# shiyao-li/NextBestPath

Hardware: AMD Instinct MI355X
Metric: exploration steps/s (+ NBP maps/s) at 256x256 (higher is better)
Workload: dtype f32

## Files before the change

### nextbestpath_amd/csrc/nbp_internal.h

```cpp
#pragma once
#include "common.h"

typedef unsigned short bf16_t;

enum { NBP_TILE_AUTO = 0, NBP_TILE_128x128 = 1, NBP_TILE_256x64 = 2, NBP_TILE_256x32 = 3, NBP_TILE_128x64 = 4,
       NBP_TILE_64x128 = 5,
       NBP_TILE_HALO_128 = 6, NBP_TILE_HALO_64 = 7,
       NBP_TILE_HALO4_128 = 8, NBP_TILE_HALO4_64 = 9,
       NBP_TILE_SPLIT_HALO_64 = 10, NBP_TILE_SPLIT_UP = 11,
       NBP_TILE_HALO_UP_128 = 12, NBP_TILE_HALO_UP_64 = 13,
       NBP_TILE_RESERVED_14 = 14,
       NBP_TILE_SPLIT_HALO_R8 = 15, NBP_TILE_SPLIT_UP_R8 = 16,
       NBP_TILE_SPLIT_UP_DGRAD = 17,
       NBP_TILE_SPLIT_HALO_128 = 18,
       NBP_TILE_SPLIT_GATE = 19 };
struct TileInfo { int bm, bn; };
struct ConvPlan { int tile; int split_k; int chunks_per_split; };

struct IgemmArgs {
    const float* src0;
    const float* src1;
    int C0, C1;
    int cc0;
    int ups;
    int H, W;
    int Hs, Ws;
    int taps;
    const float* wpk;
    int N;
    const float* scale;
    const float* shift;
    int relu;
    float* out;
    long long M;
    int split_k;
    int chunks_total;
    int chunks_per_split;
    unsigned bytes0, bytes1;
    unsigned bytesw;
    float* partial;
    int groups;
    const float* g_src0;
    const float* g_src1;
    const float* g_wpk;
    const float* g_scale;
    const float* g_shift;
    float* g_out;
    int xcd_remap;
};
struct ConvOperands { const float* src0; const float* src1; const float* wpk; const float* scale; const float* shift; float* out; };
// ... 59 lines not shown
```

### nextbestpath_amd/csrc/nbp_split.hip

```cpp
#include "common.h"
#include "nbp_internal.h"
#include <cstdlib>

namespace {

typedef _Float16 f16x8 __attribute__((ext_vector_type(8)));
typedef _Float16 f16x2 __attribute__((ext_vector_type(2)));
typedef unsigned u32x4 __attribute__((ext_vector_type(4)));
typedef unsigned u32x2 __attribute__((ext_vector_type(2)));
typedef __attribute__((address_space(3))) void* lds_ptr_t;

constexpr int SPLIT_EXP = 14;
__host__ __device__ inline int amax_exponent(unsigned bits) {
    if (!bits) return SPLIT_EXP;
    int e = (int)((bits >> 23) & 255u) - 127;
    return e < -100 ? -100 : (e > 100 ? 100 : e);
}
__host__ __device__ inline float pow2f(int e) {
    union { unsigned u; float f; } v;
    v.u = (unsigned)(127 + e) << 23;
    return v.f;
}

__device__ __forceinline__ void split_pair(float x0, float x1, unsigned& h, unsigned& l) {
// ... 17 lines not shown
}
__device__ __forceinline__ void block_amax(float mx, unsigned* out, unsigned words = AMAX_WORDS) {
    __shared__ float part[4];
#pragma unroll
    for (int o = 32; o; o >>= 1) mx = fmaxf(mx, __shfl_xor(mx, o));
    if ((threadIdx.x & 63) == 0) part[threadIdx.x >> 6] = mx;
    __syncthreads();
    if (threadIdx.x == 0)
        atomicMax(out + (blockIdx.x & (words - 1)), __float_as_uint(fmaxf(fmaxf(part[0], part[1]), fmaxf(part[2], part[3]))));
}
__device__ __forceinline__ unsigned read_amax(const unsigned* slot) {
    unsigned v = slot[threadIdx.x & (AMAX_WORDS - 1)];
#pragma unroll
    for (int o = 32; o; o >>= 1) { const unsigned u = __shfl_xor(v, o); v = u > v ? u : v; }
    return v;
}

struct SplitOps {
    const float* src0; const float* src1; const void* planes; const float* scale; const float* shift; float* out;
    const unsigned* amax0; const unsigned* amax1; const unsigned* wamax; unsigned* amax_out;
    float* pool_out;
    const float* head_w; const float* head_ss[2]; float* head_out;
    double* bn_part;
    const float* psi0;
};
struct SplitArgs {
    SplitOps g[2];
    int C0, C1, ups, H, W, Hs, Ws, N, relu;
    long long M;
    int split_k, chunks_total, chunks_per_split;
    unsigned bytes0, bytes1, bytesw;
    float* partial;
    int groups, xcd_remap;
};

#ifdef NBP_DBG_TS
__device__ unsigned long long nbp_dbg_ts[8192];
__device__ unsigned nbp_dbg_n;
#define NBP_WALL(tag) do { if (dbg_on) { const unsigned k_ = dbg_i++; if (k_ < 4000) { nbp_dbg_ts[2 * k_] = (unsigned long long)(tag); nbp_dbg_ts[2 * k_ + 1] = wall_clock64(); } } } while (0)
#define NBP_TS(tag) do { if (dbg_on) { const unsigned k_ = dbg_i++; if (k_ < 4000) { nbp_dbg_ts[2 * k_] = (unsigned long long)(tag); nbp_dbg_ts[2 * k_ + 1] = __builtin_readcyclecounter(); } } } while (0)
#else
#define NBP_TS(tag) do {} while (0)
#endif
template <bool ONE, int TW, int TM, int TN, bool PH, bool BS = false, bool P2 = false, bool DG = false>
__global__ __launch_bounds__(256, 2) __attribute__((amdgpu_waves_per_eu(2, 2))) void conv3x3_halo_h2_kernel(SplitArgs a) {
    static_assert(!P2 || PH, "two-parity form: up_conv layers");
    static_assert(!DG || (PH && !BS && !P2), "data gradient of an up_conv layer: the one-parity tap structure");
    constexpr bool PHO = PH && !DG;
    int zs = blockIdx.z;
    const int py = PHO ? (P2 ? zs & 1 : (zs >> 1) & 1) : 0, px = (PHO && !P2) ? zs & 1 : 0;
    if (PHO) zs >>= (P2 ? 1 : 2);
    const int zslice = zs;
    const SplitOps& o = zs >= a.split_k ? a.g[1] : a.g[0];
    if (zs >= a.split_k) zs -= a.split_k;
    constexpr int ROWS = PH ? 2 : 3, TPR = PH ? 2 : 3, TAPS = ROWS * TPR;
    constexpr int BN = TN * 32, NB = BN / 64;
    constexpr int RPB = 32 / TW, TH = 4 * TM * RPB;
    constexpr int HW_ = TW + 2, HPIX = (TH + 2) * HW_;
    constexpr int RS = (HPIX + 7) / 8 * 8 * 16 + 64;
    constexpr int NPL = ONE ? 1 : 2;
    constexpr int HALO_BYTES = 2 * NPL * RS;
    constexpr int WI = TPR * 2 * NPL * NB;
    constexpr int NPAR = P2 ? 2 : 1;
    constexpr int WB1 = WI * 1024, WB = NPAR * WB1;
    constexpr int NF = (HPIX * 4 + 255) / 256;
    static_assert(BN % 64 == 0 && (TH == 16 || TH == 8), "tile shape");
    extern __shared__ __attribute__((aligned(16))) char ldsb[];
    char* const halo = ldsb;
    char* const wbuf = ldsb + HALO_BYTES;
    float* const psil = reinterpret_cast<float*>(ldsb + HALO_BYTES + 2 * WB);

    const int tid = threadIdx.x, lane = tid & 63, wave = tid >> 6;
#ifdef NBP_DBG_TS
    const bool dbg_on = blockIdx.x == gridDim.x / 2 && blockIdx.y == 0 && blockIdx.z == 0 && tid == 64;
    unsigned dbg_i = 0;
    NBP_WALL(100); NBP_TS(101);
#endif
    const int Ht = PHO ? a.Hs : a.H, Wt = PHO ? a.Ws : a.W;
    const int tiles_x = Wt / TW, tiles_y = Ht / TH;
    unsigned tile = blockIdx.x, nt = blockIdx.y;
    if (a.xcd_remap == 1) {
        const unsigned L = blockIdx.x + gridDim.x * blockIdx.y, T = gridDim.x * gridDim.y;
        const unsigned xcd = L & 7u, idx = L >> 3, q = T >> 3, r = T & 7u;
        const unsigned v = xcd * q + min(xcd, r) + idx;
        nt = v % gridDim.y;
        tile = v / gridDim.y;
    } else if (a.xcd_remap == 2) {
// ... 226 lines not shown
#pragma unroll
                for (int j = 0; j < TN; ++j)
#pragma unroll
                    for (int p = 0; p < 2; ++p)
                        wp[j][p] = *reinterpret_cast<const u32x4*>(Bt + ((tt * 4 + p * 2) * NB + (j >> 1)) * 1024 + (j & 1) * 512);
                constexpr int PX[3] = {1, 0, 0};
                constexpr int PW[3] = {0, 1, 0};
#pragma unroll
                for (int v = 0; v < 3; ++v)
#pragma unroll
                    for (int j = 0; j < TN; ++j)
#pragma unroll
                        for (int i = 0; i < TM; ++i)
                            acc[i][j] = __builtin_amdgcn_mfma_f32_32x32x16_f16(__builtin_bit_cast(f16x8, xp[i][PX[v]]),
                                                                               __builtin_bit_cast(f16x8, wp[j][PW[v]]), acc[i][j], 0, 0, 0);
            }
            }
            NBP_TS(2);
            asm volatile("s_waitcnt vmcnt(0)" ::: "memory");
            NBP_TS(3);
            __syncthreads();
            NBP_TS(4);
        }
        if (more) {
            __builtin_amdgcn_s_setprio(0);
            store_halo(c + 1);
            NBP_TS(5);
            __syncthreads();
            NBP_TS(6);
            __builtin_amdgcn_s_setprio(2);
        }
    }

    const bool final_out = (a.split_k == 1);
    float* outp = final_out ? o.out : a.partial + (long long)zslice * a.M * a.N;
    float mx = 0.f;
    constexpr int PS = PHO ? 2 : 1;
    const long long e0 = (PHO ? ((long long)b * a.H + 2 * y0 + py) * a.W + 2 * x0 : ((long long)b * a.H + y0) * a.W + x0) * a.N + n0;
    const long long erem = (a.M * a.N - e0) * 4;
    const __amdgpu_buffer_rsrc_t rso = __builtin_amdgcn_make_buffer_rsrc(outp + e0, 0, erem < 0x7fffffffll ? (int)erem : 0x7fffffff, 0x00020000);
    const unsigned vout = (unsigned)(((TM * wave * RPB * PS * a.W + 4 * khalf * PS) * a.N + (lane & 31)) * 4);
    constexpr bool HEADABLE = !PH && TN == 2;
    const bool head = HEADABLE && final_out && o.head_out;
    const bool bn_stats = BS && final_out && o.bn_part;
    double* const bsh = reinterpret_cast<double*>(ldsb);
    if constexpr (BS) { if (bn_stats) __syncthreads(); }
    double bs1[BS ? TN : 1], bs2[BS ? TN : 1];
#pragma unroll
    for (int j = 0; j < (BS ? TN : 1); ++j) { bs1[j] = 0.0; bs2[j] = 0.0; }
    float hp[HEADABLE ? TM : 1][16];
    if constexpr (HEADABLE) {
#pragma unroll
        for (int i = 0; i < TM; ++i)
#pragma unroll
            for (int r = 0; r < 16; ++r) hp[i][r] = 0.f;
    }
#pragma unroll
    for (int pq = 0; pq < NPAR; ++pq)
#pragma unroll
    for (int j = 0; j < TN; ++j) {
        const int pxe = P2 ? pq : px;
        const int n = n0 + j * 32 + (lane & 31);
        float sc = 1.f, sh = 0.f;
        if (final_out) { sc = o.scale[n]; sh = o.shift[n]; }
        const float hw = head ? o.head_w[n] : 0.f;
        float vals[TM][16];
#pragma unroll
        for (int i = 0; i < TM; ++i) {
#pragma unroll
            for (int r = 0; r < 16; ++r) {
                const int q = (r & 3) + 8 * (r >> 2);
                const unsigned soff = (unsigned)((((i * RPB + q / TW) * PS * a.W + (q % TW) * PS + (PHO ? pxe : 0)) * a.N + j * 32) * 4);
                float v = ldexpf(accs[pq][i][j][r], einv) * sc + sh;
                if (final_out && a.relu) v = fmaxf(v, 0.f);
                mx = fmaxf(mx, fabsf(v));
                if (!head) __builtin_amdgcn_raw_buffer_store_b32(__builtin_bit_cast(unsigned, v), rso, vout, soff, 0);
                vals[i][r] = v;
                if constexpr (HEADABLE) hp[i][r] = fmaf(v, hw, hp[i][r]);
            }
        }
        if constexpr (BS) {
            if (bn_stats) {
#pragma unroll
                for (int i = 0; i < TM; ++i)
#pragma unroll
                    for (int r = 0; r < 16; ++r) { const double d = (double)vals[i][r]; bs1[j] += d; bs2[j] = fma(d, d, bs2[j]); }
            }
        }
        if (!PH && final_out && o.pool_out) {
            const int Hp = a.H >> 1, Wp = a.W >> 1;
            if constexpr (TW == 32) {
#pragma unroll
                for (int i = 0; i < TM; i += 2) {
                    const long long prow = ((long long)b * Hp + ((y0 + TM * wave + i) >> 1)) * Wp + (x0 >> 1);
#pragma unroll
                    for (int r = 0; r < 16; r += 2) {
                        const int xo = ((r & 3) + 8 * (r >> 2) + 4 * khalf) >> 1;
                        o.pool_out[(prow + xo) * a.N + n] = fmaxf(fmaxf(vals[i][r], vals[i][r + 1]), fmaxf(vals[i + 1][r], vals[i + 1][r + 1]));
                    }
                }
            } else {
#pragma unroll
                for (int i = 0; i < TM; ++i) {
                    const long long prow = ((long long)b * Hp + ((y0 + (TM * wave + i) * RPB) >> 1)) * Wp + (x0 >> 1);
#pragma unroll
                    for (int r = 0; r < 8; r += 2) {
// ... 681 lines not shown
    const unsigned stride = gridDim.x * 256u * 4u;
    float mx = 0.f;
    for (unsigned i0 = (blockIdx.x * 256u + threadIdx.x) * 4u; i0 < MN; i0 += 2 * stride) {
        const unsigned i1 = i0 + stride;
        const bool two = i1 < MN;
        f32x4 v0 = *reinterpret_cast<const f32x4*>(partial + i0);
        f32x4 v1 = two ? *reinterpret_cast<const f32x4*>(partial + i1) : f32x4{0.f, 0.f, 0.f, 0.f};
        for (int s0 = 1; s0 < split_k; s0 += 4) {
            f32x4 u0[4], u1[4];
#pragma unroll
            for (int k = 0; k < 4; ++k) {
                const bool in = s0 + k < split_k;
                const float* ps = partial + (size_t)(s0 + k) * MN;
                u0[k] = in ? *reinterpret_cast<const f32x4*>(ps + i0) : f32x4{0.f, 0.f, 0.f, 0.f};
                u1[k] = in && two ? *reinterpret_cast<const f32x4*>(ps + i1) : f32x4{0.f, 0.f, 0.f, 0.f};
            }
#pragma unroll
            for (int k = 0; k < 4; ++k)
                if (s0 + k < split_k) {
#pragma unroll
                    for (int e = 0; e < 4; ++e) { v0[e] += u0[k][e]; v1[e] += u1[k][e]; }
                }
        }
#pragma unroll
        for (int h = 0; h < 2; ++h) {
            if (h && !two) break;
            const unsigned i = h ? i1 : i0;
            f32x4 v = h ? v1 : v0;
            const unsigned n = i % N;
            const f32x4 sc = *reinterpret_cast<const f32x4*>(scale + n);
            const f32x4 sh = *reinterpret_cast<const f32x4*>(shift + n);
#pragma unroll
            for (int e = 0; e < 4; ++e) {
                v[e] = v[e] * sc[e] + sh[e];
                if (relu) v[e] = fmaxf(v[e], 0.f);
                mx = fmaxf(mx, fabsf(v[e]));
            }
            *reinterpret_cast<f32x4*>(out + i) = v;
        }
    }
    if (amax_out) block_amax(mx, amax_out);
}

__global__ __launch_bounds__(256) void splitk_reduce_pool_kernel(const float* __restrict__ partial, int split_k, unsigned MN, unsigned N,
                                                                 int H, int W, SplitOps o, int relu) {
    const unsigned N4 = N >> 2, Wp = (unsigned)W >> 1, Hp = (unsigned)H >> 1;
    const unsigned total = (MN >> 4);
    const unsigned rowN = (unsigned)W * N;
    float mx = 0.f;
    for (unsigned p = blockIdx.x * 256u + threadIdx.x; p < total; p += gridDim.x * 256u) {
        const unsigned n4 = p % N4;
        unsigned q = p / N4;
        const unsigned xp = q % Wp; q /= Wp;
        const unsigned yp = q % Hp, b = q / Hp;
        const unsigned base = ((b * (unsigned)H + 2u * yp) * (unsigned)W + 2u * xp) * N + 4u * n4;
        const unsigned idx[4] = {base, base + N, base + rowN, base + rowN + N};
        f32x4 v[4];
#pragma unroll
        for (int k = 0; k < 4; ++k) v[k] = *reinterpret_cast<const f32x4*>(partial + idx[k]);
        for (int s0 = 1; s0 < split_k; s0 += 2) {
            f32x4 u[2][4];
#pragma unroll
            for (int t = 0; t < 2; ++t) {
                const bool in = s0 + t < split_k;
                const float* ps = partial + (size_t)(s0 + t) * MN;
#pragma unroll
                for (int k = 0; k < 4; ++k) u[t][k] = in ? *reinterpret_cast<const f32x4*>(ps + idx[k]) : f32x4{0.f, 0.f, 0.f, 0.f};
            }
#pragma unroll
            for (int t = 0; t < 2; ++t)
                if (s0 + t < split_k) {
#pragma unroll
                    for (int k = 0; k < 4; ++k)
#pragma unroll
                        for (int e = 0; e < 4; ++e) v[k][e] += u[t][k][e];
                }
        }
        const f32x4 sc = *reinterpret_cast<const f32x4*>(o.scale + 4u * n4);
        const f32x4 sh = *reinterpret_cast<const f32x4*>(o.shift + 4u * n4);
        f32x4 pm;
#pragma unroll
        for (int k = 0; k < 4; ++k) {
#pragma unroll
            for (int e = 0; e < 4; ++e) {
                float r = v[k][e] * sc[e] + sh[e];
                if (relu) r = fmaxf(r, 0.f);
                mx = fmaxf(mx, fabsf(r));
                v[k][e] = r;
                pm[e] = k ? fmaxf(pm[e], r) : r;
            }
            *reinterpret_cast<f32x4*>(o.out + idx[k]) = v[k];
        }
        *reinterpret_cast<f32x4*>(o.pool_out + 4u * p) = pm;
    }
    if (o.amax_out) block_amax(mx, o.amax_out);
}

__global__ __launch_bounds__(256) void amax_kernel(const float* __restrict__ x, long long n, const float* __restrict__ row_scale,
                                                   long long per_row, unsigned* __restrict__ out, unsigned words) {
    float mx = 0.f;
    if (!row_scale && (n & 3) == 0 && ((uintptr_t)x & 15) == 0) {
        for (long long i = (long long)blockIdx.x * blockDim.x + threadIdx.x; i < n / 4; i += (long long)gridDim.x * blockDim.x) {
            const f32x4 v = reinterpret_cast<const f32x4*>(x)[i];
            mx = fmaxf(fmaxf(mx, fmaxf(fabsf(v[0]), fabsf(v[1]))), fmaxf(fabsf(v[2]), fabsf(v[3])));
        }
    } else {
        for (long long i = (long long)blockIdx.x * blockDim.x + threadIdx.x; i < n; i += (long long)gridDim.x * blockDim.x)
            mx = fmaxf(mx, fabsf(row_scale ? x[i] * row_scale[i / per_row] : x[i]));
    }
    block_amax(mx, out, words);
}

template <bool ONE = false>
__global__ void pack_conv_weight_h2_kernel(const float* __restrict__ w, int N, int C, int taps, const float* __restrict__ scale,
                                           int c_off, const unsigned* __restrict__ wamax, unsigned short* __restrict__ dst,
                                           int transposed = 0) {
    const float sw = pow2f(SPLIT_EXP - amax_exponent(*wamax));
    const long long total = (long long)N * C * taps;
// ... 204 lines not shown
            constexpr int NPL = ONE ? 1 : 2;
            e.planes = d.planes + (long long)ph * (C >> 4) * 4 * 2 * NPL * N * 8;
            if (d.planes_t) e.planes_t = d.planes_t + (long long)ph * (N >> 4) * 4 * 2 * NPL * C * 8;
            prepack_store_block<ONE>(e, hl, n8, c8, tap, d.planes_t ? (1 - r) * 2 + (1 - tt) : -1, 4);
        }
        return;
    }
    const int taps = d.kind == 0 ? 9 : 1;
    const long long total = (long long)N8 * C8 * taps;
    for (long long i = (long long)blockIdx.x * blockDim.x + threadIdx.x; i < total; i += (long long)gridDim.x * blockDim.x) {
        const int tap = (int)(i % taps);
        const long long t = i / taps;
        const int c8 = (int)(t % C8), n8 = (int)(t / C8);
        unsigned hl[8][8];
#pragma unroll
        for (int nn = 0; nn < 8; ++nn)
#pragma unroll
            for (int cc = 0; cc < 8; ++cc) {
                unsigned h, l;
                split_pair(d.w[((long long)(n8 * 8 + nn) * C + c8 * 8 + cc) * taps + tap] * swf, 0.f, h, l);
                hl[nn][cc] = (h & 0xffffu) | (l << 16);
            }
        prepack_store_block<ONE>(d, hl, n8, c8, tap, d.planes_t ? taps - 1 - tap : -1, taps);
    }
}

int split_tile_width(int H, int W, int N, int ksize) {
    if (ksize != 3 || H < 16 || H % 16) return 0;
    if (W >= 32 && W % 32 == 0 && N % 64 == 0) return 32;
    if (W >= 16 && W % 16 == 0 && N % 128 == 0) return 16;
    return 0;
}

template <int TW, int TM, int TN, bool PH, bool BS = false, bool P2 = false, bool DG = false, bool ONE = false>
int launch_h2(const SplitArgs& a, hipStream_t st, int tile) {
    {
        char nm[96];
        snprintf(nm, sizeof(nm), "conv3x3_halo_h2_kernel<%s, %d, %d, %d, %s, %s, %s, %s>", ONE ? "true" : "false", TW, TM, TN, PH ? "true" : "false",
                 BS ? "true" : "false", P2 ? "true" : "false", DG ? "true" : "false");
        nbp_note_kernel_symbol(tile, nm);
    }
    constexpr int TH = 4 * TM * (32 / TW);
    constexpr int HPIX = (TH + 2) * (TW + 2), RS = (HPIX + 7) / 8 * 8 * 16 + 64, NB = TN / 2;
    constexpr int NPL = ONE ? 1 : 2;
    constexpr size_t smem = 2 * NPL * (size_t)RS + 2 * (size_t)(PH ? 4 : 6) * NPL * NB * 1024 * (P2 ? 2 : 1) + (PH ? 0 : (HPIX * 4 + 15) / 16 * 16);
    static bool attr_set = false;
    if (!attr_set) {
        hipError_t e = hipFuncSetAttribute(reinterpret_cast<const void*>(&conv3x3_halo_h2_kernel<ONE, TW, TM, TN, PH, BS, P2, DG>),
                                           hipFuncAttributeMaxDynamicSharedMemorySize, (int)smem);
        if (e != hipSuccess) return (int)e;
        attr_set = true;
    }
    constexpr bool PHO = PH && !DG;
    NBP_RETURN_IF((long long)(2 * TH + 2) * a.W * a.N * 4 >= (1ll << 31), NBP_E_SHAPE);
    dim3 grid((unsigned)(a.M / (PHO ? 4 : 1) / (TH * TW)), (unsigned)(a.N / (TN * 32)), (unsigned)(a.split_k * a.groups * (PHO ? (P2 ? 2 : 4) : 1)));
    conv3x3_halo_h2_kernel<ONE, TW, TM, TN, PH, BS, P2, DG><<<grid, 256, smem, st>>>(a);
    return nbp_launch_status();
}
template <int TW, int TM, int TN, bool PH, bool BS = false, bool P2 = false, bool DG = false>
int launch_h2o(const SplitArgs& a, hipStream_t st, int tile, int one) {
    return one ? launch_h2<TW, TM, TN, PH, BS, P2, DG, true>(a, st, tile) : launch_h2<TW, TM, TN, PH, BS, P2, DG, false>(a, st, tile);
}

}

static int chain_bounded_split(int sk, int cc, int taps, long long M, int N, int groups) {
    static const int max_k = nbp_tune_int("NBP_SPLIT_MAX_K", NBP_SPLIT_MAX_K_DEFAULT);
    static const int max_k_small = nbp_tune_int("NBP_SPLIT_MAX_K_SMALL", NBP_SPLIT_MAX_K_SMALL_DEFAULT);
    const bool small = (double)M * N * groups * 4.0 <= 64.0 * 1048576.0;
    const int mk = small && max_k_small > 0 ? max_k_small : max_k;
    if (mk <= 0) return sk;
    const int max_chunks = mk / (16 * taps) > 1 ? mk / (16 * taps) : 1;
    const int need = (int)nbp_cdiv(cc, max_chunks);
    return need > sk ? need : sk;
}

static long long half_rows_below() {
    static const int v = nbp_tune_int("NBP_SPLIT_R8_BLOCKS", 256);
    return v;
}


static bool half_rows_for_tail(long long workgroups) {
    if (workgroups <= 512) return false;
    const long long rem = workgroups % 512;
    return rem > 0 && rem <= 160;
}

ConvPlan nbp_plan_conv_split(long long M, int N, int chunks_total, int split_k, int groups, int H, int W, int ksize, int ups) {
    ConvPlan p{0, 1, chunks_total};
    constexpr int min_blocks = 256;
    if (ups && !((H | W) & 1)) {
        const int twu = split_tile_width(H / 2, W / 2, N, ksize);
        if (twu) {
            const int cc = chunks_total / 9 * 2;
            const long long blocks = (M / 4 / (16 * twu)) * (N / (twu == 32 ? 64 : 128)) * groups * 4;
            const bool r8 = blocks < half_rows_below();
            int sk = split_k;
            if (sk <= 0) {
                sk = 1;
                while (blocks * sk < min_blocks && cc / (sk * 2) >= 4 && sk < 16) sk *= 2;
            }
            if (split_k == 0) sk = chain_bounded_split(sk, cc, 4, M, N, groups);
            if (sk > cc) sk = cc;
            const int per = (int)nbp_cdiv(cc, sk);
            p.split_k = (int)nbp_cdiv(cc, per); p.chunks_per_split = per;
            const bool r8t = r8 || half_rows_for_tail((M / 4 / (16 * twu)) * (N / (twu == 32 ? 64 : 128)) * groups * 4 * p.split_k);
            p.tile = r8t ? NBP_TILE_SPLIT_UP_R8 : NBP_TILE_SPLIT_UP;
            return p;
        }
    }
    const int tw = split_tile_width(H, W, N, ksize);
    if (!tw) return p;
    const int cc = chunks_total / 9 * 2;
    const long long blocks = (M / (16 * tw)) * (N / (tw == 32 ? 64 : 128)) * groups;
    const bool r8 = blocks < half_rows_below();
    int sk = split_k;
    if (sk <= 0) {
        sk = 1;
        while (blocks * sk < min_blocks && cc / (sk * 2) >= 4 && sk < 16) sk *= 2;
        if (blocks * sk < 2 * min_blocks && cc / (sk * 2) >= 16 && sk < 16) sk *= 2;
        if (split_k == 0) sk = chain_bounded_split(sk, cc, 9, M, N, groups);
    }
    if (sk > cc) sk = cc;
    const int per = (int)nbp_cdiv(cc, sk);
    p.split_k = (int)nbp_cdiv(cc, per); p.chunks_per_split = per;
    const bool r8t = r8 || half_rows_for_tail((M / (16 * tw)) * (N / (tw == 32 ? 64 : 128)) * groups * p.split_k);
    p.tile = r8t ? NBP_TILE_SPLIT_HALO_R8 : (tw == 32 && N % 128 == 0) ? NBP_TILE_SPLIT_HALO_128 : NBP_TILE_SPLIT_HALO_64;
    return p;
}

int nbp_amax_launch(const float* x, long long n, unsigned* amax_inout, hipStream_t st) {
    if (n <= 0) return 0;
    amax_kernel<<<min(nbp_ew_grid(n / 4 + 1, 256), 1024), 256, 0, st>>>(x, n, nullptr, 1, amax_inout, AMAX_WORDS);
    return nbp_launch_status();
}

int nbp_conv_split_launch_g(const ConvOperandsSplit& o, const ConvOperandsSplit* o2, int C0, int C1, int ups, int B, int H, int W,
                            int ksize, int N, int relu, int split_k, void* ws, size_t ws_bytes, hipStream_t st,
                            float* const* pool_out, int* pooled, const ConvHead* head, int* headed, double* bn_part, int* bn_rows, int one) {
    const int groups = o2 ? 2 : 1;
    if (bn_rows) *bn_rows = 0;
    NBP_RETURN_IF(!o.src0 || !o.planes || !o.scale || !o.shift || !o.out || !o.amax0 || !o.wamax, NBP_E_ARG);
    NBP_RETURN_IF(o2 && (!o2->src0 || !o2->planes || !o2->scale || !o2->shift || !o2->out || !o2->amax0 || !o2->wamax), NBP_E_ARG);
    NBP_RETURN_IF(B < 1 || H < 1 || W < 1 || ksize != 3, NBP_E_ARG);
    NBP_RETURN_IF(C0 < 32 || C0 % 32 || C1 < 0 || C1 % 32 || N < 64 || N % 64, NBP_E_SHAPE);
    NBP_RETURN_IF(C1 > 0 && (!o.src1 || !o.amax1 || (o2 && (!o2->src1 || !o2->amax1))), NBP_E_ARG);
    NBP_RETURN_IF(ups && ((H | W) & 1), NBP_E_SHAPE);
    SplitArgs a;
    for (int g = 0; g < 2; ++g) {
        const ConvOperandsSplit& s = (g && o2) ? *o2 : o;
        a.g[g] = SplitOps{s.src0, s.src1, s.planes, s.scale, s.shift, s.out, s.amax0, C1 ? s.amax1 : nullptr, s.wamax, s.amax_out, nullptr, nullptr, {nullptr, nullptr}, nullptr, nullptr, s.psi0};
    }
    NBP_RETURN_IF((o.psi0 || (o2 && o2->psi0)) && ups, NBP_E_SHAPE);
    a.C0 = C0; a.C1 = C1; a.ups = ups ? 1 : 0;
    a.H = H; a.W = W; a.Hs = ups ? H / 2 : H; a.Ws = ups ? W / 2 : W;
    a.N = N; a.relu = relu; a.groups = groups;
    a.M = (long long)B * H * W;
    const long long b0 = (long long)B * a.Hs * a.Ws * C0 * 4, b1 = (long long)B * a.Hs * a.Ws * C1 * 4;
    const long long bw = (long long)(C0 + C1) * 9 * N * 4;
    NBP_RETURN_IF(b0 >= (1ll << 31) || b1 >= (1ll << 31) || bw >= (1ll << 31), NBP_E_SHAPE);
    a.bytes0 = (unsigned)b0; a.bytes1 = C1 ? (unsigned)b1 : (unsigned)b0; a.bytesw = (unsigned)bw;
    const bool have_up = ups && o.planes_up && o.wamax_up && (!o2 || (o2->planes_up && o2->wamax_up));
    const ConvPlan p = nbp_plan_conv_split(a.M, N, (C0 + C1) / 32 * 9, split_k, groups, H, W, ksize, have_up ? 1 : 0);
    NBP_RETURN_IF(p.tile != NBP_TILE_SPLIT_HALO_64 && p.tile != NBP_TILE_SPLIT_HALO_128 && p.tile != NBP_TILE_SPLIT_UP && p.tile != NBP_TILE_SPLIT_HALO_R8 &&
                  p.tile != NBP_TILE_SPLIT_UP_R8, NBP_E_SHAPE);
    const bool ph = p.tile == NBP_TILE_SPLIT_UP || p.tile == NBP_TILE_SPLIT_UP_R8;
    const bool r8 = p.tile == NBP_TILE_SPLIT_HALO_R8 || p.tile == NBP_TILE_SPLIT_UP_R8;
    const bool wide = p.tile == NBP_TILE_SPLIT_HALO_128;
    const int th = (r8 || wide) ? 8 : 16;
    a.split_k = p.split_k; a.chunks_per_split = p.chunks_per_split;
    a.chunks_total = (C0 + C1) / 16;
    const int tw = ph ? split_tile_width(H / 2, W / 2, N, ksize) : split_tile_width(H, W, N, ksize);
    if (ph) {
        NBP_RETURN_IF(C1 != 0, NBP_E_SHAPE);
        for (int g = 0; g < groups; ++g) {
            const ConvOperandsSplit& sg = (g && o2) ? *o2 : o;
            a.g[g].planes = sg.planes_up; a.g[g].wamax = sg.wamax_up;
        }
        const long long bwu = (long long)C0 * 16 * N * 4;
        NBP_RETURN_IF(bwu >= (1ll << 31), NBP_E_SHAPE);
        a.bytesw = (unsigned)bwu;
    }
    {
        const long long ptiles = a.M / (ph ? 4 : 1) / (th * tw), nbk = N / ((tw == 32 && !wide) ? 64 : 128);
        const long long tiles = ptiles * nbk;
        const double wb = (double)(C0 + C1) * (ph ? 16 : 9) * N * 4, ab = (double)a.M / (ups ? 4 : 1) * (C0 + C1) * 4;
        const bool fits2 = nbk >= 8 ? nbk % 8 == 0 : (8 % nbk == 0 && ptiles % (8 / nbk) == 0);
        const bool heavy = 7.0 * wb > ((nbk < 8 ? nbk : 8) - 1) * ab * 3.0;
        int mode = tiles >= 8 ? 1 : 0;
        if (fits2 && heavy && tiles >= 8) mode = 2;
        a.xcd_remap = mode;
    }
    a.partial = nullptr;
    if (p.split_k > 1) {
        NBP_RETURN_IF(!ws || ws_bytes < (size_t)groups * p.split_k * a.M * N * sizeof(float), NBP_E_WS);
        a.partial = (float*)ws;
    }
    static const int allow_pool = nbp_tune_int("NBP_CONV_POOL", 1);
    const bool with_pool = allow_pool && pool_out && pool_out[0] && (groups == 1 || pool_out[1]) && p.split_k == 1 && !ph && !ups &&
                           !((H | W) & 1);
    const bool pool_in_reduce = allow_pool && pool_out && pool_out[0] && groups == 1 && p.split_k > 1 && !ph && !ups && !((H | W) & 1);
    if (pooled) *pooled = with_pool || pool_in_reduce;
    if (with_pool || pool_in_reduce)
        for (int g = 0; g < groups; ++g) a.g[g].pool_out = pool_out[g];
    static const int allow_head = nbp_tune_int("NBP_CONV_HEAD", 1);
    const bool with_head = allow_head && head && head->w && head->scale && head->shift && head->out && groups == 1 && p.split_k == 1 &&
                           !ph && tw == 32 && N == 64 && relu;
    if (headed) *headed = with_head;
    if (with_head) { a.g[0].head_w = head->w; a.g[0].head_ss[0] = head->scale; a.g[0].head_ss[1] = head->shift; a.g[0].head_out = head->out; }
    if (bn_part && bn_rows && p.split_k == 1 && !r8 && groups == 1) {
        a.g[0].bn_part = bn_part;
        *bn_rows = (int)(a.M / (16 * tw));
        if (wide) {
            *bn_rows = (int)(a.M / 256);
            return launch_h2o<32, 2, 4, false, true>(a, st, p.tile, one);
        }
        return ph ? (tw == 32 ? launch_h2o<32, 2, 2, true, true, true>(a, st, p.tile, one) : launch_h2o<16, 2, 4, true, true>(a, st, p.tile, one))
                  : (tw == 32 ? launch_h2o<32, 4, 2, false, true>(a, st, p.tile, one) : launch_h2o<16, 2, 4, false, true>(a, st, p.tile, one));
    }
    int rc = (ph && !r8 && tw == 32) ? launch_h2o<32, 2, 2, true, false, true>(a, st, p.tile, one)
           : r8 ? (ph ? (tw == 32 ? launch_h2o<32, 2, 2, true>(a, st, p.tile, one) : launch_h2o<16, 1, 4, true>(a, st, p.tile, one))
                      : (tw == 32 ? launch_h2o<32, 2, 2, false>(a, st, p.tile, one) : launch_h2o<16, 1, 4, false>(a, st, p.tile, one)))
           : ph ? launch_h2o<16, 2, 4, true>(a, st, p.tile, one)
                : (tw == 32 ? (wide ? launch_h2o<32, 2, 4, false>(a, st, p.tile, one) : launch_h2o<32, 4, 2, false>(a, st, p.tile, one))
                            : launch_h2o<16, 2, 4, false>(a, st, p.tile, one));
    if (rc) return rc;
    if (p.split_k > 1) {
        const long long MN = a.M * N;
        NBP_RETURN_IF(MN >= (1ll << 31), NBP_E_SHAPE);
        dim3 grid((unsigned)min(nbp_cdiv(MN / 4, 256 * 4), 1024ll), (unsigned)groups);
        if (pool_in_reduce)
            splitk_reduce_pool_kernel<<<(unsigned)min(nbp_cdiv(MN / 16, 256), 1024ll), 256, 0, st>>>((const float*)ws, p.split_k, (unsigned)MN,
                                                                                                    (unsigned)N, H, W, a.g[0], relu);
        else
        splitk_reduce_split_kernel<<<grid, 256, 0, st>>>((const float*)ws, p.split_k, (unsigned)MN, (unsigned)N, a.g[0], a.g[1], relu);
        rc = nbp_launch_status();
    }
    return rc;
}

int nbp_pack_conv_weight_split_launch(const float* w_oihw, int N, int C, int ksize, const float* scale_or_null, int c_off,
                                      int c_total, void* dst, unsigned* wamax_out, hipStream_t st, int one) {
    NBP_RETURN_IF(!w_oihw || !dst || !wamax_out, NBP_E_ARG);
    NBP_RETURN_IF(ksize != 1 && ksize != 3, NBP_E_ARG);
    NBP_RETURN_IF(N < 1 || C < 1 || c_off != 0 || C > c_total || c_total % 32, NBP_E_SHAPE);
    const long long total = (long long)N * C * ksize * ksize;
    hipError_t e = hipMemsetAsync(wamax_out, 0, sizeof(unsigned), st);
    if (e != hipSuccess) return (int)e;
    amax_kernel<<<min(nbp_ew_grid(total, 256), 256), 256, 0, st>>>(w_oihw, total, scale_or_null, (long long)C * ksize * ksize, wamax_out, 1u);
    const int grid = nbp_ew_grid(total, 256);
    if (one) pack_conv_weight_h2_kernel<true><<<grid, 256, 0, st>>>(w_oihw, N, C, ksize * ksize, scale_or_null, c_off, wamax_out, (unsigned short*)dst);
    else pack_conv_weight_h2_kernel<<<grid, 256, 0, st>>>(w_oihw, N, C, ksize * ksize, scale_or_null, c_off, wamax_out, (unsigned short*)dst);
    return nbp_launch_status();
}

int nbp_pack_upconv_weight_split_launch(const float* w_oihw, int N, int C, void* dst, unsigned* wamax_out, hipStream_t st, int one) {
    NBP_RETURN_IF(!w_oihw || !dst || !wamax_out, NBP_E_ARG);
    NBP_RETURN_IF(N < 1 || C < 16 || C % 16, NBP_E_SHAPE);
// ... 60 lines not shown
    }
    if (with_psi) {
        if (bn == 128) gate1x1_h2_kernel<false, 4, true><<<grid, 256, smem, st>>>(a);
        else if (bn == 64) gate1x1_h2_kernel<false, 2, true><<<grid, 256, smem, st>>>(a);
        else gate1x1_h2_kernel<false, 1, true><<<grid, 256, smem, st>>>(a);
    } else if (bn == 128) gate1x1_h2_kernel<false, 4, false><<<grid, 256, smem, st>>>(a);
    else if (bn == 64) gate1x1_h2_kernel<false, 2, false><<<grid, 256, smem, st>>>(a);
    else gate1x1_h2_kernel<false, 1, false><<<grid, 256, smem, st>>>(a);
    return nbp_launch_status();
}

int nbp_upconv_dgrad_split_launch(const float* dy, int N, int B, int H, int W, const void* planes, const unsigned* wamax,
                                  const unsigned* amax_in, int C, const float* scale, const float* shift, float* out, unsigned* amax_out,
                                  int split_k, void* ws, size_t ws_bytes, hipStream_t st, int one = 0) {
    NBP_RETURN_IF(!dy || !planes || !wamax || !amax_in || !scale || !shift || !out, NBP_E_ARG);
    NBP_RETURN_IF(B < 1 || N < 16 || N % 16 || C < 64 || C % 64, NBP_E_SHAPE);
    const int tw = split_tile_width(H, W, C, 3);
    NBP_RETURN_IF(!tw, NBP_E_SHAPE);
    SplitArgs a;
    for (int g = 0; g < 2; ++g)
        a.g[g] = SplitOps{dy, nullptr, planes, scale, shift, out, amax_in, nullptr, wamax, amax_out, nullptr, nullptr, {nullptr, nullptr}, nullptr, nullptr};
    a.C0 = N; a.C1 = 0; a.ups = 0; a.H = H; a.W = W; a.Hs = 2 * H; a.Ws = 2 * W; a.N = C; a.relu = 0; a.groups = 1;
    a.M = (long long)B * H * W;
    const long long b0 = (long long)B * 4 * H * W * N * 4, bw = 64ll * N * C;
    NBP_RETURN_IF(b0 >= (1ll << 31) || bw >= (1ll << 31), NBP_E_SHAPE);
    a.bytes0 = (unsigned)b0; a.bytes1 = (unsigned)b0; a.bytesw = (unsigned)bw;
    a.chunks_total = 4 * (N / 16);
    const long long blocks = (a.M / ((tw == 32 ? 8 : 16) * tw)) * (C / (tw == 32 ? 64 : 128));
    int sk = split_k;
    if (sk <= 0) { sk = 1; while (blocks * sk < 256 && a.chunks_total / (sk * 2) >= 4 && sk < 16) sk *= 2; }
    if (sk > a.chunks_total) sk = a.chunks_total;
    a.chunks_per_split = (int)nbp_cdiv(a.chunks_total, sk);
    a.split_k = (int)nbp_cdiv(a.chunks_total, a.chunks_per_split);
    a.xcd_remap = blocks >= 8 ? 1 : 0;
    a.partial = nullptr;
    if (a.split_k > 1) {
        NBP_RETURN_IF(!ws || ws_bytes < (size_t)a.split_k * a.M * C * sizeof(float), NBP_E_WS);
        a.partial = (float*)ws;
    }
    int rc = tw == 32 ? launch_h2o<32, 2, 2, true, false, false, true>(a, st, NBP_TILE_SPLIT_UP_DGRAD, one)
                      : launch_h2o<16, 2, 4, true, false, false, true>(a, st, NBP_TILE_SPLIT_UP_DGRAD, one);
    if (rc) return rc;
    if (a.split_k > 1) {
        const long long MN = a.M * C;
        NBP_RETURN_IF(MN >= (1ll << 31), NBP_E_SHAPE);
        dim3 grid((unsigned)min(nbp_cdiv(MN / 4, 256 * 4), 1024ll), 1u);
        splitk_reduce_split_kernel<<<grid, 256, 0, st>>>((const float*)ws, a.split_k, (unsigned)MN, (unsigned)C, a.g[0], a.g[1], 0);
        rc = nbp_launch_status();
    }
    return rc;
}

int nbp_conv1x1_split_launch(const float* src, int C, long long M, const void* planes, const unsigned* wamax, const unsigned* amax_in,
                             int N, const float* scale, const float* shift, int relu, float* out, hipStream_t st, int one = 0) {
    NBP_RETURN_IF(!src || !planes || !wamax || !amax_in || !scale || !shift || !out, NBP_E_ARG);
    NBP_RETURN_IF(C < 32 || C % 32 || N < 32 || N % 32 || M < 1, NBP_E_SHAPE);
    const long long b0 = M * C * 4, bw = (long long)C * N * 4;
    NBP_RETURN_IF(b0 >= (1ll << 31) || bw >= (1ll << 31) || M * N * 4 >= (1ll << 33), NBP_E_SHAPE);
    GateArgs a;
    for (int g = 0; g < 2; ++g) {
        a.g[g] = SplitOps{src, nullptr, planes, scale, shift, out, amax_in, nullptr, wamax, nullptr, nullptr, nullptr, {nullptr, nullptr}, nullptr, nullptr};
        a.wpsi[g] = nullptr; a.st[g] = nullptr; a.gated[g] = nullptr; a.gated_amax[g] = nullptr;
    }
    a.C = C; a.C1 = 0; a.N = N; a.relu = relu; a.M = M; a.bytes0 = (unsigned)b0; a.bytesw = (unsigned)bw; a.groups = 1;
    int bn = N % 128 == 0 ? 128 : (N % 64 == 0 ? 64 : 32);
    if (bn == 128 && nbp_cdiv(M, 128) * (N / 128) < 512) bn = 64;
// ... 466 lines not shown
```

Baseline: 2371.

## Fuse split-K reduction into a finishing launch of the last K slice

For split-K halo convolutions, the first split_k-1 slices now write partials, and a second launch computes the last slice and sums the earlier partial planes in its epilogue before applying scale, shift, ReLU and pooling. This removes the separate split-K reduce kernel and one write/read of a partial plane. In exchange the last slice runs as its own serialized launch with fewer workgroups, which is why it is gated on a minimum workgroup count. A few epilogues also switch to fmaf.

```diff
diff --git a/nextbestpath_amd/csrc/nbp_internal.h b/nextbestpath_amd/csrc/nbp_internal.h
--- a/nextbestpath_amd/csrc/nbp_internal.h
+++ b/nextbestpath_amd/csrc/nbp_internal.h
@@ -15,7 +15,7 @@
        NBP_TILE_SPLIT_HALO_128 = 18,
        NBP_TILE_SPLIT_GATE = 19 };
 struct TileInfo { int bm, bn; };
-struct ConvPlan { int tile; int split_k; int chunks_per_split; };
+struct ConvPlan { int tile; int split_k; int chunks_per_split; int finish; };
 
 struct IgemmArgs {
     const float* src0;
diff --git a/nextbestpath_amd/csrc/nbp_split.hip b/nextbestpath_amd/csrc/nbp_split.hip
--- a/nextbestpath_amd/csrc/nbp_split.hip
+++ b/nextbestpath_amd/csrc/nbp_split.hip
@@ -73,6 +73,7 @@
     unsigned bytes0, bytes1, bytesw;
     float* partial;
     int groups, xcd_remap;
+    int slice0, slices, finish;
 };
 
 #ifdef NBP_DBG_TS
@@ -83,17 +84,20 @@
 #else
 #define NBP_TS(tag) do {} while (0)
 #endif
-template <bool ONE, int TW, int TM, int TN, bool PH, bool BS = false, bool P2 = false, bool DG = false>
+template <bool FIN, bool ONE, int TW, int TM, int TN, bool PH, bool BS = false, bool P2 = false, bool DG = false>
 __global__ __launch_bounds__(256, 2) __attribute__((amdgpu_waves_per_eu(2, 2))) void conv3x3_halo_h2_kernel(SplitArgs a) {
     static_assert(!P2 || PH, "two-parity form: up_conv layers");
     static_assert(!DG || (PH && !BS && !P2), "data gradient of an up_conv layer: the one-parity tap structure");
+    static_assert(!FIN || (!BS && !DG), "finishing launches: the inference forms");
     constexpr bool PHO = PH && !DG;
     int zs = blockIdx.z;
     const int py = PHO ? (P2 ? zs & 1 : (zs >> 1) & 1) : 0, px = (PHO && !P2) ? zs & 1 : 0;
     if (PHO) zs >>= (P2 ? 1 : 2);
-    const int zslice = zs;
-    const SplitOps& o = zs >= a.split_k ? a.g[1] : a.g[0];
-    if (zs >= a.split_k) zs -= a.split_k;
+    const int zgroup = zs >= a.slices ? 1 : 0;
+    const SplitOps& o = zgroup ? a.g[1] : a.g[0];
+    if (zgroup) zs -= a.slices;
+    zs += a.slice0;
+    const int zslice = zgroup * a.split_k + zs;
     constexpr int ROWS = PH ? 2 : 3, TPR = PH ? 2 : 3, TAPS = ROWS * TPR;
     constexpr int BN = TN * 32, NB = BN / 64;
     constexpr int RPB = 32 / TW, TH = 4 * TM * RPB;
@@ -386,7 +390,7 @@
         }
     }
 
-    const bool final_out = (a.split_k == 1);
+    const bool final_out = FIN || a.split_k == 1;
     float* outp = final_out ? o.out : a.partial + (long long)zslice * a.M * a.N;
     float mx = 0.f;
     constexpr int PS = PHO ? 2 : 1;
@@ -394,7 +398,25 @@
     const long long erem = (a.M * a.N - e0) * 4;
     const __amdgpu_buffer_rsrc_t rso = __builtin_amdgcn_make_buffer_rsrc(outp + e0, 0, erem < 0x7fffffffll ? (int)erem : 0x7fffffff, 0x00020000);
     const unsigned vout = (unsigned)(((TM * wave * RPB * PS * a.W + 4 * khalf * PS) * a.N + (lane & 31)) * 4);
-    constexpr bool HEADABLE = !PH && TN == 2;
+    constexpr bool HEADABLE = !PH && TN == 2 && !FIN;
+    const float* const prev0 = FIN ? a.partial + (long long)zgroup * a.split_k * a.M * a.N + e0 : nullptr;
+    const int prev_bytes = erem < 0x7fffffffll ? (int)erem : 0x7fffffff;
+    const int nprev = a.slice0;
+    auto soff_of = [&](int pq, int j, int i, int r) {
+        const int q = (r & 3) + 8 * (r >> 2);
+        return (unsigned)((((i * RPB + q / TW) * PS * a.W + (q % TW) * PS + (PHO ? (P2 ? pq : px) : 0)) * a.N + j * 32) * 4);
+    };
+    auto plane = [&](int s) {
+        return __builtin_amdgcn_make_buffer_rsrc(const_cast<float*>(prev0 + (long long)s * a.M * a.N), 0, prev_bytes, 0x00020000);
+    };
+    auto load_slice = [&](__amdgpu_buffer_rsrc_t rs, float (&dst)[16], int pq, int j, int i) {
+#pragma unroll
+        for (int r = 0; r < 16; ++r) dst[r] = __builtin_bit_cast(float, __builtin_amdgcn_raw_buffer_load_b32(rs, vout, soff_of(pq, j, i, r), 0));
+    };
+    const __amdgpu_buffer_rsrc_t rp0 = plane(0);
+    float pre[16];
+    constexpr int SPB = (TW == 16 && TM == 2 && !PH) ? 1 : 2;
+    if constexpr (FIN) load_slice(rp0, pre, 0, 0, 0);
     const bool head = HEADABLE && final_out && o.head_out;
     const bool bn_stats = BS && final_out && o.bn_part;
     double* const bsh = reinterpret_cast<double*>(ldsb);
@@ -413,7 +435,6 @@
     for (int pq = 0; pq < NPAR; ++pq)
 #pragma unroll
     for (int j = 0; j < TN; ++j) {
-        const int pxe = P2 ? pq : px;
         const int n = n0 + j * 32 + (lane & 31);
         float sc = 1.f, sh = 0.f;
         if (final_out) { sc = o.scale[n]; sh = o.shift[n]; }
@@ -421,11 +442,31 @@
         float vals[TM][16];
 #pragma unroll
         for (int i = 0; i < TM; ++i) {
+            float prev[FIN ? 16 : 1];
+            if constexpr (FIN) {
+#pragma unroll
+                for (int r = 0; r < 16; ++r) prev[r] = pre[r];
+                const int ni = i + 1 < TM ? i + 1 : 0, nj = ni ? j : (j + 1 < TN ? j + 1 : 0), npq = (ni || nj) ? pq : pq + 1;
+                if (npq < NPAR) load_slice(rp0, pre, npq, nj, ni);
+                for (int s = 1; s < nprev; s += SPB) {
+                    float u[SPB][16];
+#pragma unroll
+                    for (int t = 0; t < SPB; ++t)
+                        if (s + t < nprev) load_slice(plane(s + t), u[t], pq, j, i);
+#pragma unroll
+                    for (int t = 0; t < SPB; ++t)
+                        if (s + t < nprev) {
+#pragma unroll
+                            for (int r = 0; r < 16; ++r) prev[r] += u[t][r];
+                        }
+                }
+            }
 #pragma unroll
             for (int r = 0; r < 16; ++r) {
-                const int q = (r & 3) + 8 * (r >> 2);
-                const unsigned soff = (unsigned)((((i * RPB + q / TW) * PS * a.W + (q % TW) * PS + (PHO ? pxe : 0)) * a.N + j * 32) * 4);
-                float v = ldexpf(accs[pq][i][j][r], einv) * sc + sh;
+                const unsigned soff = soff_of(pq, j, i, r);
+                float v;
+                if constexpr (FIN) v = fmaf(prev[r] + ldexpf(accs[pq][i][j][r], einv), sc, sh);
+                else v = ldexpf(accs[pq][i][j][r], einv) * sc + sh;
                 if (final_out && a.relu) v = fmaxf(v, 0.f);
                 mx = fmaxf(mx, fabsf(v));
                 if (!head) __builtin_amdgcn_raw_buffer_store_b32(__builtin_bit_cast(unsigned, v), rso, vout, soff, 0);
@@ -1173,7 +1214,7 @@
             const f32x4 sh = *reinterpret_cast<const f32x4*>(shift + n);
 #pragma unroll
             for (int e = 0; e < 4; ++e) {
-                v[e] = v[e] * sc[e] + sh[e];
+                v[e] = fmaf(v[e], sc[e], sh[e]);
                 if (relu) v[e] = fmaxf(v[e], 0.f);
                 mx = fmaxf(mx, fabsf(v[e]));
             }
@@ -1224,7 +1265,7 @@
         for (int k = 0; k < 4; ++k) {
 #pragma unroll
             for (int e = 0; e < 4; ++e) {
-                float r = v[k][e] * sc[e] + sh[e];
+                float r = fmaf(v[k][e], sc[e], sh[e]);
                 if (relu) r = fmaxf(r, 0.f);
                 mx = fmaxf(mx, fabsf(r));
                 v[k][e] = r;
@@ -1495,11 +1536,11 @@
     return 0;
 }
 
-template <int TW, int TM, int TN, bool PH, bool BS = false, bool P2 = false, bool DG = false, bool ONE = false>
+template <int TW, int TM, int TN, bool PH, bool BS = false, bool P2 = false, bool DG = false, bool ONE = false, bool FIN = false>
 int launch_h2(const SplitArgs& a, hipStream_t st, int tile) {
-    {
+    if (!FIN) {
         char nm[96];
-        snprintf(nm, sizeof(nm), "conv3x3_halo_h2_kernel<%s, %d, %d, %d, %s, %s, %s, %s>", ONE ? "true" : "false", TW, TM, TN, PH ? "true" : "false",
+        snprintf(nm, sizeof(nm), "conv3x3_halo_h2_kernel<false, %s, %d, %d, %d, %s, %s, %s, %s>", ONE ? "true" : "false", TW, TM, TN, PH ? "true" : "false",
                  BS ? "true" : "false", P2 ? "true" : "false", DG ? "true" : "false");
         nbp_note_kernel_symbol(tile, nm);
     }
@@ -1509,20 +1550,27 @@
     constexpr size_t smem = 2 * NPL * (size_t)RS + 2 * (size_t)(PH ? 4 : 6) * NPL * NB * 1024 * (P2 ? 2 : 1) + (PH ? 0 : (HPIX * 4 + 15) / 16 * 16);
     static bool attr_set = false;
     if (!attr_set) {
-        hipError_t e = hipFuncSetAttribute(reinterpret_cast<const void*>(&conv3x3_halo_h2_kernel<ONE, TW, TM, TN, PH, BS, P2, DG>),
+        hipError_t e = hipFuncSetAttribute(reinterpret_cast<const void*>(&conv3x3_halo_h2_kernel<FIN, ONE, TW, TM, TN, PH, BS, P2, DG>),
                                            hipFuncAttributeMaxDynamicSharedMemorySize, (int)smem);
         if (e != hipSuccess) return (int)e;
         attr_set = true;
     }
     constexpr bool PHO = PH && !DG;
     NBP_RETURN_IF((long long)(2 * TH + 2) * a.W * a.N * 4 >= (1ll << 31), NBP_E_SHAPE);
-    dim3 grid((unsigned)(a.M / (PHO ? 4 : 1) / (TH * TW)), (unsigned)(a.N / (TN * 32)), (unsigned)(a.split_k * a.groups * (PHO ? (P2 ? 2 : 4) : 1)));
-    conv3x3_halo_h2_kernel<ONE, TW, TM, TN, PH, BS, P2, DG><<<grid, 256, smem, st>>>(a);
+    NBP_RETURN_IF(a.slices < 1 || a.slice0 < 0 || a.slice0 + a.slices > a.split_k, NBP_E_ARG);
+    NBP_RETURN_IF(FIN != (a.finish != 0) || (FIN && (a.slices != 1 || a.slice0 < 1 || !a.partial)), NBP_E_ARG);
+    dim3 grid((unsigned)(a.M / (PHO ? 4 : 1) / (TH * TW)), (unsigned)(a.N / (TN * 32)), (unsigned)(a.slices * a.groups * (PHO ? (P2 ? 2 : 4) : 1)));
+    conv3x3_halo_h2_kernel<FIN, ONE, TW, TM, TN, PH, BS, P2, DG><<<grid, 256, smem, st>>>(a);
     return nbp_launch_status();
 }
 template <int TW, int TM, int TN, bool PH, bool BS = false, bool P2 = false, bool DG = false>
 int launch_h2o(const SplitArgs& a, hipStream_t st, int tile, int one) {
     return one ? launch_h2<TW, TM, TN, PH, BS, P2, DG, true>(a, st, tile) : launch_h2<TW, TM, TN, PH, BS, P2, DG, false>(a, st, tile);
+}
+template <int TW, int TM, int TN, bool PH, bool P2 = false>
+int launch_h2f(const SplitArgs& a, hipStream_t st, int tile, int one) {
+    if (!a.finish) return launch_h2o<TW, TM, TN, PH, false, P2>(a, st, tile, one);
+    return one ? launch_h2<TW, TM, TN, PH, false, P2, false, true, true>(a, st, tile) : launch_h2<TW, TM, TN, PH, false, P2, false, false, true>(a, st, tile);
 }
 
 }
@@ -1550,8 +1598,16 @@
     return rem > 0 && rem <= 160;
 }
 
+static int finish_by_rule(int request, int split_k, long long last_slice_wgs) {
+    static const int mode = nbp_tune_int("NBP_SPLIT_FINISH", 1);
+    static const int min_wgs = nbp_tune_int("NBP_SPLIT_FINISH_MIN_WGS", 512);
+    if (split_k < 2 || mode <= 0) return 0;
+    if (mode >= 2) return 1;
+    return request == 0 && last_slice_wgs >= min_wgs ? 1 : 0;
+}
+
 ConvPlan nbp_plan_conv_split(long long M, int N, int chunks_total, int split_k, int groups, int H, int W, int ksize, int ups) {
-    ConvPlan p{0, 1, chunks_total};
+    ConvPlan p{0, 1, chunks_total, 0};
     constexpr int min_blocks = 256;
     if (ups && !((H | W) & 1)) {
         const int twu = split_tile_width(H / 2, W / 2, N, ksize);
@@ -1570,6 +1626,7 @@
             p.split_k = (int)nbp_cdiv(cc, per); p.chunks_per_split = per;
             const bool r8t = r8 || half_rows_for_tail((M / 4 / (16 * twu)) * (N / (twu == 32 ? 64 : 128)) * groups * 4 * p.split_k);
             p.tile = r8t ? NBP_TILE_SPLIT_UP_R8 : NBP_TILE_SPLIT_UP;
+            p.finish = finish_by_rule(split_k, p.split_k, blocks * (r8t ? 2 : 1));
             return p;
         }
     }
@@ -1590,6 +1647,7 @@
     p.split_k = (int)nbp_cdiv(cc, per); p.chunks_per_split = per;
     const bool r8t = r8 || half_rows_for_tail((M / (16 * tw)) * (N / (tw == 32 ? 64 : 128)) * groups * p.split_k);
     p.tile = r8t ? NBP_TILE_SPLIT_HALO_R8 : (tw == 32 && N % 128 == 0) ? NBP_TILE_SPLIT_HALO_128 : NBP_TILE_SPLIT_HALO_64;
+    p.finish = finish_by_rule(split_k, p.split_k, blocks * (r8t ? 2 : 1));
     return p;
 }
 
@@ -1633,7 +1691,9 @@
     const bool wide = p.tile == NBP_TILE_SPLIT_HALO_128;
     const int th = (r8 || wide) ? 8 : 16;
     a.split_k = p.split_k; a.chunks_per_split = p.chunks_per_split;
+    a.slice0 = 0; a.slices = p.split_k; a.finish = 0;
     a.chunks_total = (C0 + C1) / 16;
+    const bool finish = p.finish && p.split_k > 1 && !bn_part;
     const int tw = ph ? split_tile_width(H / 2, W / 2, N, ksize) : split_tile_width(H, W, N, ksize);
     if (ph) {
         NBP_RETURN_IF(C1 != 0, NBP_E_SHAPE);
@@ -1661,9 +1721,9 @@
         a.partial = (float*)ws;
     }
     static const int allow_pool = nbp_tune_int("NBP_CONV_POOL", 1);
-    const bool with_pool = allow_pool && pool_out && pool_out[0] && (groups == 1 || pool_out[1]) && p.split_k == 1 && !ph && !ups &&
+    const bool with_pool = allow_pool && pool_out && pool_out[0] && (groups == 1 || pool_out[1]) && (p.split_k == 1 || finish) && !ph && !ups &&
                            !((H | W) & 1);
-    const bool pool_in_reduce = allow_pool && pool_out && pool_out[0] && groups == 1 && p.split_k > 1 && !ph && !ups && !((H | W) & 1);
+    const bool pool_in_reduce = allow_pool && pool_out && pool_out[0] && groups == 1 && p.split_k > 1 && !finish && !ph && !ups && !((H | W) & 1);
     if (pooled) *pooled = with_pool || pool_in_reduce;
     if (with_pool || pool_in_reduce)
         for (int g = 0; g < groups; ++g) a.g[g].pool_out = pool_out[g];
@@ -1682,12 +1742,22 @@
         return ph ? (tw == 32 ? launch_h2o<32, 2, 2, true, true, true>(a, st, p.tile, one) : launch_h2o<16, 2, 4, true, true>(a, st, p.tile, one))
                   : (tw == 32 ? launch_h2o<32, 4, 2, false, true>(a, st, p.tile, one) : launch_h2o<16, 2, 4, false, true>(a, st, p.tile, one));
     }
-    int rc = (ph && !r8 && tw == 32) ? launch_h2o<32, 2, 2, true, false, true>(a, st, p.tile, one)
-           : r8 ? (ph ? (tw == 32 ? launch_h2o<32, 2, 2, true>(a, st, p.tile, one) : launch_h2o<16, 1, 4, true>(a, st, p.tile, one))
-                      : (tw == 32 ? launch_h2o<32, 2, 2, false>(a, st, p.tile, one) : launch_h2o<16, 1, 4, false>(a, st, p.tile, one)))
-           : ph ? launch_h2o<16, 2, 4, true>(a, st, p.tile, one)
-                : (tw == 32 ? (wide ? launch_h2o<32, 2, 4, false>(a, st, p.tile, one) : launch_h2o<32, 4, 2, false>(a, st, p.tile, one))
-                            : launch_h2o<16, 2, 4, false>(a, st, p.tile, one));
+    auto launch = [&](const SplitArgs& a) {
+        return (ph && !r8 && tw == 32) ? launch_h2f<32, 2, 2, true, true>(a, st, p.tile, one)
+           : r8 ? (ph ? (tw == 32 ? launch_h2f<32, 2, 2, true>(a, st, p.tile, one) : launch_h2f<16, 1, 4, true>(a, st, p.tile, one))
+                      : (tw == 32 ? launch_h2f<32, 2, 2, false>(a, st, p.tile, one) : launch_h2f<16, 1, 4, false>(a, st, p.tile, one)))
+           : ph ? launch_h2f<16, 2, 4, true>(a, st, p.tile, one)
+                : (tw == 32 ? (wide ? launch_h2f<32, 2, 4, false>(a, st, p.tile, one) : launch_h2f<32, 4, 2, false>(a, st, p.tile, one))
+                            : launch_h2f<16, 2, 4, false>(a, st, p.tile, one));
+    };
+    if (finish) {
+        a.slices = p.split_k - 1;
+        int rc = launch(a);
+        if (rc) return rc;
+        a.slice0 = p.split_k - 1; a.slices = 1; a.finish = 1;
+        return launch(a);
+    }
+    int rc = launch(a);
     if (rc) return rc;
     if (p.split_k > 1) {
         const long long MN = a.M * N;
@@ -1814,6 +1884,7 @@
     if (sk > a.chunks_total) sk = a.chunks_total;
     a.chunks_per_split = (int)nbp_cdiv(a.chunks_total, sk);
     a.split_k = (int)nbp_cdiv(a.chunks_total, a.chunks_per_split);
+    a.slice0 = 0; a.slices = a.split_k; a.finish = 0;
     a.xcd_remap = blocks >= 8 ? 1 : 0;
     a.partial = nullptr;
     if (a.split_k > 1) {
```

Result: faster. 2400 (median of 6 runs) (+1.2%).
